# WestlyPark/StyleRenderer

Measured on AMD Instinct MI355X. Metric: generator fwd+bwd images/sec at 256^2, higher is better.
Workload: dtype f32

## Files before the change

### stylerenderer_amd/csrc/fused_elem.hip

```cpp
#include "common.h"

namespace {

constexpr int EB = 256;
constexpr int ECHUNK = EB * 16;

__device__ __forceinline__ void block_sum2(float& a, float& b, float* lds8) {
    a = sr_wave_sum(a);
    b = sr_wave_sum(b);
    const int lane = threadIdx.x & 63, wave = threadIdx.x >> 6;
    if (lane == 0) { lds8[wave] = a; lds8[4 + wave] = b; }
    __syncthreads();
    if (threadIdx.x == 0) {
        a = (lds8[0] + lds8[1]) + (lds8[2] + lds8[3]);
        b = (lds8[4] + lds8[5]) + (lds8[6] + lds8[7]);
    }
}

template <bool REF>
__global__ __launch_bounds__(EB) void k_nba_fwd(float* __restrict__ y, const float* __restrict__ x,
                                                const float* __restrict__ noise,
                                                const float* __restrict__ noise_w,
                                                const float* __restrict__ bias,
                                                const float* __restrict__ ref, float alpha, float scale,
// ... 114 lines not shown
}

template <bool SCALE_OUT, bool VEC>
__global__ __launch_bounds__(EB) void k_rowdot(float* __restrict__ partial, float* __restrict__ out,
                                               const float* __restrict__ a, const float* __restrict__ b,
                                               const float* __restrict__ s, int64_t inner, int chunks,
                                               const float* __restrict__ rdiv) {
    __shared__ float lds8[8];
    const int64_t row = blockIdx.y;
    const int64_t off = (int64_t)blockIdx.x * ECHUNK;
    const int64_t remain = inner - off;
    const int n = (int)(remain < ECHUNK ? remain : ECHUNK);
    const float sc = SCALE_OUT ? s[row] : 1.0f;
    float acc = 0.0f, dummy = 0.0f;
    if (VEC) {
        const float4* as = reinterpret_cast<const float4*>(a + row * inner + off);
        const float4* bs = reinterpret_cast<const float4*>(b + row * inner + off);
        float4* os = SCALE_OUT ? reinterpret_cast<float4*>(out + row * inner + off) : nullptr;
        for (int i = threadIdx.x; i < n / 4; i += EB) {
            const float4 x = as[i], y = bs[i];
            acc += (x.x * y.x + x.y * y.y) + (x.z * y.z + x.w * y.w);
            if (SCALE_OUT) os[i] = make_float4(y.x * sc, y.y * sc, y.z * sc, y.w * sc);
        }
    } else {
        const float* as = a + row * inner + off;
        const float* bs = b + row * inner + off;
        float* os = SCALE_OUT ? out + row * inner + off : nullptr;
#pragma unroll 4
        for (int i = threadIdx.x; i < n; i += EB) {
            const float x = as[i], y = bs[i];
            acc += x * y;
            if (SCALE_OUT) os[i] = y * sc;
        }
    }
    block_sum2(acc, dummy, lds8);
    if (threadIdx.x == 0) partial[row * chunks + blockIdx.x] = rdiv ? acc / rdiv[row] : acc;
}

__global__ __launch_bounds__(64) void k_rowdot_finish(float* __restrict__ dots,
                                                      const float* __restrict__ partial, int chunks,
                                                      const float* __restrict__ rdiv = nullptr) {
    const int64_t row = blockIdx.x;
    float acc = 0.0f;
    for (int i = threadIdx.x; i < chunks; i += 64) acc += partial[row * chunks + i];
    acc = sr_wave_sum(acc);
    if (threadIdx.x == 0) dots[row] = rdiv ? acc / rdiv[row] : acc;
}

inline bool vec_ok(int64_t inner, const void* p0, const void* p1, const void* p2, const void* p3) {
    const uintptr_t m = (uintptr_t)p0 | (uintptr_t)p1 | (uintptr_t)p2 | (uintptr_t)p3;
    return inner % 4 == 0 && (m & 15) == 0;
}

}

extern "C" int sr_noise_bias_act(float* y, const float* x, const float* noise, const float* noise_w,
                                 const float* bias, const float* ref, float alpha, float scale,
                                 int64_t n, int64_t c, int64_t inner, int64_t noise_bstride,
                                 sr_stream_t stream) {
    if (n < 0 || c < 0 || inner < 0) return SR_EINVAL;
    if (n * c * inner == 0) return SR_OK;
    if (!y || !x || (noise && !noise_w) || n * c > 65535) return SR_EINVAL;
    if (!vec_ok(inner, y, x, noise, ref) || (noise && noise_bstride % 4 != 0)) return SR_EINVAL;
    const int chunks = (int)sr_ceil_div(inner, ECHUNK);
    const dim3 grid(chunks, (unsigned)(n * c));
    hipStream_t st = sr_stream(stream);
    if (ref)
        hipLaunchKernelGGL(k_nba_fwd<true>, grid, dim3(EB), 0, st, y, x, noise, noise_w, bias, ref, alpha,
                           scale, (int)c, inner, noise_bstride);
    else
        hipLaunchKernelGGL(k_nba_fwd<false>, grid, dim3(EB), 0, st, y, x, noise, noise_w, bias, ref, alpha,
                           scale, (int)c, inner, noise_bstride);
    return sr_launch_status();
}

extern "C" int64_t sr_noise_bias_act_bwd_scratch_floats(int64_t n, int64_t c, int64_t inner) {
    if (n <= 0 || c <= 0 || inner <= 0) return 2;
    return 2 * n * c * sr_ceil_div(inner, ECHUNK) + c + 2;
}

extern "C" int sr_noise_bias_act_bwd(float* gx, float* gbias, float* gnoise_w, const float* gy,
                                     const float* out, const float* noise, float alpha, float scale,
                                     int64_t n, int64_t c, int64_t inner, int64_t noise_bstride,
                                     float* scratch, sr_stream_t stream) {
    if (n < 0 || c < 0 || inner < 0) return SR_EINVAL;
    if (n * c * inner == 0) return SR_OK;
    if (!gx || !gy || !out || !scratch || n * c > 65535) return SR_EINVAL;
    if (!vec_ok(inner, gx, gy, out, noise) || (noise && noise_bstride % 4 != 0)) return SR_EINVAL;
    const int chunks = (int)sr_ceil_div(inner, ECHUNK);
    hipStream_t st = sr_stream(stream);
    hipLaunchKernelGGL(k_nba_bwd<false>, dim3(chunks, (unsigned)(n * c)), dim3(EB), 0, st, gx, scratch, gy, out,
                       noise, alpha, scale, (int)c, inner, noise_bstride, chunks, (const float*)nullptr,
                       (const float*)nullptr, 0.0f, 0.0f, (float*)nullptr);
    float* chan_nw = scratch + 2 * n * c * (int64_t)chunks;
    if (gbias) {
        hipLaunchKernelGGL(k_nba_finish, dim3((unsigned)c), dim3(64), 0, st, gbias, chan_nw, scratch, n, (int)c,
                           chunks);
        if (noise && gnoise_w)
            hipLaunchKernelGGL(k_nba_finish2, dim3(1), dim3(64), 0, st, gnoise_w, chan_nw, (int)c);
    }
    return sr_launch_status();
}

int sr_nba_finish_launch(float* gbias, float* gnoise_w, float* rowdot, const float* partial, const float* dot_partial,
                         float* chan_nw, int64_t n, int64_t c, int chunks, bool has_noise, hipStream_t st) {
    if (gbias) {
        hipLaunchKernelGGL(k_nba_finish, dim3((unsigned)c), dim3(64), 0, st, gbias, chan_nw, partial, n, (int)c, chunks);
        if (has_noise && gnoise_w)
            hipLaunchKernelGGL(k_nba_finish2, dim3(1), dim3(64), 0, st, gnoise_w, chan_nw, (int)c);
    }
    if (rowdot) hipLaunchKernelGGL(k_rowdot_finish, dim3((unsigned)(n * c)), dim3(64), 0, st, rowdot, dot_partial, chunks);
    return sr_launch_status();
}

extern "C" int64_t sr_noise_bias_act_bwd_dot_scratch_floats(int64_t n, int64_t c, int64_t inner) {
    if (n <= 0 || c <= 0 || inner <= 0) return 3;
    return 3 * n * c * sr_ceil_div(inner, ECHUNK) + c + 2;
}

extern "C" int sr_noise_bias_act_bwd_dot(float* gx, float* gbias, float* gnoise_w, float* rowdot, const float* gy,
                                         const float* out, const float* noise, const float* noise_w,
                                         const float* bias, float alpha, float scale, int64_t n, int64_t c,
                                         int64_t inner, int64_t noise_bstride, float* scratch,
                                         sr_stream_t stream) {
    if (n < 0 || c < 0 || inner < 0) return SR_EINVAL;
    if (n * c * inner == 0) return SR_OK;
    if (!gx || !gy || !out || !scratch || !rowdot || n * c > 65535 || (noise && !noise_w) || scale == 0.0f ||
        alpha == 0.0f)
        return SR_EINVAL;
    if (!vec_ok(inner, gx, gy, out, noise) || (noise && noise_bstride % 4 != 0)) return SR_EINVAL;
    const int chunks = (int)sr_ceil_div(inner, ECHUNK);
    hipStream_t st = sr_stream(stream);
    float* dot_scratch = scratch + 2 * n * c * (int64_t)chunks;
    float* chan_nw = dot_scratch + n * c * (int64_t)chunks;
    float* dot_partial = chunks == 1 ? rowdot : dot_scratch;
    hipLaunchKernelGGL(k_nba_bwd<true>, dim3(chunks, (unsigned)(n * c)), dim3(EB), 0, st, gx, scratch, gy, out, noise,
                       alpha, scale, (int)c, inner, noise_bstride, chunks, noise_w, bias, 1.0f / scale,
                       1.0f / (alpha * scale), dot_partial);
    if (gbias) {
        hipLaunchKernelGGL(k_nba_finish, dim3((unsigned)c), dim3(64), 0, st, gbias, chan_nw, scratch, n, (int)c, chunks);
        if (noise && gnoise_w)
            hipLaunchKernelGGL(k_nba_finish2, dim3(1), dim3(64), 0, st, gnoise_w, chan_nw, (int)c);
    }
    if (chunks > 1)
        hipLaunchKernelGGL(k_rowdot_finish, dim3((unsigned)(n * c)), dim3(64), 0, st, rowdot, dot_partial, chunks);
    return sr_launch_status();
}

namespace {

constexpr int APIX = EB * 4;

__global__ __launch_bounds__(EB) void k_nba_aff_fwd(float* __restrict__ y, const float* __restrict__ x,
                                                    const float* __restrict__ amap, const float* __restrict__ smap,
                                                    int64_t map_bstride, const float* __restrict__ noise,
                                                    const float* __restrict__ noise_w,
                                                    const float* __restrict__ bias, float alpha, float scale, int c,
                                                    int64_t inner, int64_t noise_bstride, int cgroup) {
    const int64_t b = blockIdx.y;
    const int64_t p = (int64_t)blockIdx.x * APIX + threadIdx.x * 4;
    if (p >= inner) return;
    const int c0 = blockIdx.z * cgroup, c1 = (c0 + cgroup < c) ? c0 + cgroup : c;
    const float4 a = *reinterpret_cast<const float4*>(amap + b * map_bstride + p);
    const float4 sft = *reinterpret_cast<const float4*>(smap + b * map_bstride + p);
    const float nw = noise ? noise_w[0] : 0.0f;
    float4 nz = make_float4(0.f, 0.f, 0.f, 0.f);
    if (noise) nz = *reinterpret_cast<const float4*>(noise + b * noise_bstride + p);
    nz.x *= nw; nz.y *= nw; nz.z *= nw; nz.w *= nw;
    for (int ch = c0; ch < c1; ++ch) {
        const int64_t o = (b * c + ch) * inner + p;
        float4 v = *reinterpret_cast<const float4*>(x + o);
        const float bb = bias ? bias[ch] : 0.0f;
        v.x = v.x * a.x + sft.x; v.y = v.y * a.y + sft.y; v.z = v.z * a.z + sft.z; v.w = v.w * a.w + sft.w;
        if (noise) { v.x += nz.x; v.y += nz.y; v.z += nz.z; v.w += nz.w; }
        v.x += bb; v.y += bb; v.z += bb; v.w += bb;
        float4 r;
        r.x = ((v.x > 0.0f) ? v.x : v.x * alpha) * scale;
        r.y = ((v.y > 0.0f) ? v.y : v.y * alpha) * scale;
        r.z = ((v.z > 0.0f) ? v.z : v.z * alpha) * scale;
        r.w = ((v.w > 0.0f) ? v.w : v.w * alpha) * scale;
        *reinterpret_cast<float4*>(y + o) = r;
    }
}

__global__ __launch_bounds__(EB) void k_nba_aff_bwd(float* __restrict__ gx, float* __restrict__ gamap,
                                                    float* __restrict__ gsmap, float* __restrict__ partial,
                                                    const float* __restrict__ gy, const float* __restrict__ out,
                                                    const float* __restrict__ x, const float* __restrict__ amap,
                                                    int64_t map_bstride, const float* __restrict__ noise,
                                                    float alpha, float scale, int c, int64_t inner,
                                                    int64_t noise_bstride, int chunks, int cgroup,
                                                    int64_t plane) {
    const int64_t b = blockIdx.y;
    const int64_t p = (int64_t)blockIdx.x * APIX + threadIdx.x * 4;
    const bool live = p < inner;
    const int c0 = blockIdx.z * cgroup, c1 = (c0 + cgroup < c) ? c0 + cgroup : c;
    gamap += (int64_t)blockIdx.z * plane;
    gsmap += (int64_t)blockIdx.z * plane;
    const int lane = threadIdx.x & 63, wave = threadIdx.x >> 6;
// ... 506 lines not shown
    }
    const int lane = threadIdx.x & 63, wave = threadIdx.x >> 6;
#pragma unroll
    for (int k = 0; k < CH; ++k)
#pragma unroll
        for (int j = 0; j < N; ++j) {
            const float r = sr_wave_sum(acc[k][j]);
            if (lane == 0) lds[k][j * 4 + wave] = r;
        }
    if (sum_g) {
#pragma unroll
        for (int j = 0; j < N; ++j) {
            const float r = sr_wave_sum(ag[j]);
            if (lane == 0) lds_g[j * 4 + wave] = r;
        }
    }
    __syncthreads();
    if (sum_g && threadIdx.x >= 64 && threadIdx.x < 64 + N) {
        const int j = threadIdx.x - 64;
        gsum[(b * chunks + blockIdx.x) * N + j] = (lds_g[j * 4] + lds_g[j * 4 + 1]) + (lds_g[j * 4 + 2] + lds_g[j * 4 + 3]);
    }
    if (threadIdx.x < CH * N) {
        const int k = threadIdx.x / N, j = threadIdx.x % N;
        const float r = (lds[k][j * 4] + lds[k][j * 4 + 1]) + (lds[k][j * 4 + 2] + lds[k][j * 4 + 3]);
        if (dws) dws[(b * N + j) * C + (row0 + k - b * C)] = r;
        else partial[((row0 + k) * chunks + blockIdx.x) * N + j] = r;
    }
}

__global__ __launch_bounds__(64) void k_smallconv_dw_finish(float* __restrict__ dws,
                                                            const float* __restrict__ partial, int C, int N,
                                                            int chunks, int64_t rows) {
    const int64_t row = blockIdx.x;
    if (row >= rows) return;
    const int64_t b = row / C, c = row % C;
    for (int j = 0; j < N; ++j) {
        float acc = 0.0f;
        for (int i = threadIdx.x; i < chunks; i += 64) acc += partial[(row * chunks + i) * N + j];
        acc = sr_wave_sum(acc);
        if (threadIdx.x == 0) dws[(b * N + j) * C + c] = acc;
    }
}

__global__ __launch_bounds__(64) void k_smallconv_gb_finish(float* __restrict__ gb, const float* __restrict__ gsum, int N,
                                                            int entries) {
    for (int j = 0; j < N; ++j) {
        float acc = 0.0f;
        for (int i = threadIdx.x; i < entries; i += 64) acc += gsum[(int64_t)i * N + j];
        acc = sr_wave_sum(acc);
        if (threadIdx.x == 0) gb[j] = acc;
    }
}

inline bool smallconv_ok(int64_t B, int64_t C, int64_t N, int64_t hw, const void* a, const void* b2) {
    return B > 0 && B <= 65535 && C > 0 && C <= 4096 && N >= 1 && N <= SC_MAXN && hw % 4 == 0 &&
           (((uintptr_t)a | (uintptr_t)b2) & 15) == 0;
}

}

#define SR_SMALLCONV_DISPATCH(KERNEL, ...)                                   \
    switch (N) {                                                             \
        case 1: hipLaunchKernelGGL(KERNEL<1>, __VA_ARGS__); break;           \
        case 2: hipLaunchKernelGGL(KERNEL<2>, __VA_ARGS__); break;           \
        case 3: hipLaunchKernelGGL(KERNEL<3>, __VA_ARGS__); break;           \
        default: hipLaunchKernelGGL(KERNEL<4>, __VA_ARGS__); break;          \
    }

extern "C" int sr_smallconv_fwd(float* out, const float* x, const float* ws, const float* bias, int64_t B,
                                int64_t C, int64_t N, int64_t hw, sr_stream_t stream) {
    if (!out || !x || !ws || !smallconv_ok(B, C, N, hw, out, x)) return SR_EINVAL;
    const int64_t hw4 = hw / 4;
    const dim3 grid((unsigned)sr_ceil_div(hw4, 64), (unsigned)B);
    hipStream_t st = sr_stream(stream);
    const bool wide = sr_ceil_div(hw4, 64) * B < 1024 && C >= 64;
#define SR_SMALLCONV_FWD(NN)                                                                                          \
    if (wide) hipLaunchKernelGGL((k_smallconv_fwd<NN, 16>), grid, dim3(1024), 0, st, out, x, ws, bias, (int)C, hw4);  \
    else hipLaunchKernelGGL((k_smallconv_fwd<NN, 4>), grid, dim3(256), 0, st, out, x, ws, bias, (int)C, hw4);
    switch (N) {
        case 1: SR_SMALLCONV_FWD(1) break;
        case 2: SR_SMALLCONV_FWD(2) break;
        case 3: SR_SMALLCONV_FWD(3) break;
        default: SR_SMALLCONV_FWD(4) break;
    }
#undef SR_SMALLCONV_FWD
    return sr_launch_status();
}

extern "C" int sr_smallconv_dx_add(float* dx, const float* g, const float* ws, const float* addend, int64_t B, int64_t C,
                                   int64_t N, int64_t hw, sr_stream_t stream);

extern "C" int sr_smallconv_dx(float* dx, const float* g, const float* ws, int64_t B, int64_t C, int64_t N,
                               int64_t hw, sr_stream_t stream) {
    return sr_smallconv_dx_add(dx, g, ws, nullptr, B, C, N, hw, stream);
}

extern "C" int sr_smallconv_dx_add(float* dx, const float* g, const float* ws, const float* addend, int64_t B, int64_t C,
                                   int64_t N, int64_t hw, sr_stream_t stream) {
    if (!dx || !g || !ws || !smallconv_ok(B, C, N, hw, dx, g) || ((uintptr_t)addend & 15)) return SR_EINVAL;
    const int64_t hw4 = hw / 4;
    const int64_t wgs = sr_ceil_div(hw4, 256) * B;
    int64_t groups = sr_ceil_div(2048, wgs);
    if (groups > sr_ceil_div(C, 8)) groups = sr_ceil_div(C, 8);
    if (groups < 1) groups = 1;
    const int cgroup = (int)(sr_ceil_div(sr_ceil_div(C, groups), 8) * 8);
    const dim3 grid((unsigned)sr_ceil_div(hw4, 256), (unsigned)B, (unsigned)sr_ceil_div(C, cgroup));
    const size_t lds = (size_t)N * C * sizeof(float);
    hipStream_t st = sr_stream(stream);
    SR_SMALLCONV_DISPATCH(k_smallconv_dx, grid, dim3(256), lds, st, dx, g, ws, (int)C, hw4, addend, cgroup);
    return sr_launch_status();
}

extern "C" int64_t sr_smallconv_dw_scratch_floats(int64_t B, int64_t C, int64_t N, int64_t hw) {
    if (B <= 0 || C <= 0 || N <= 0 || hw <= 0) return 1;
    return B * C * sr_ceil_div(hw, ECHUNK) * N + B * sr_ceil_div(hw, ECHUNK) * N + 1;
}

extern "C" int sr_smallconv_dw_bias(float* dws, float* gb, const float* g, const float* x, int64_t B, int64_t C, int64_t N,
                                    int64_t hw, float* scratch, sr_stream_t stream) {
    if (!dws || !g || !x || !scratch || !smallconv_ok(B, C, N, hw, g, x) || B * C > 65535) return SR_EINVAL;
    const int chunks = (int)sr_ceil_div(hw, ECHUNK);
    hipStream_t st = sr_stream(stream);
    float* direct = chunks == 1 ? dws : nullptr;
    float* gsum = gb ? scratch + B * C * chunks * N : nullptr;
    if (C % 4 == 0) {
        const dim3 grid((unsigned)chunks, (unsigned)(B * C / 4));
        switch (N) {
            case 1: hipLaunchKernelGGL((k_smallconv_dw<1, 4>), grid, dim3(256), 0, st, scratch, g, x, (int)C, hw, chunks, direct, gsum); break;
            case 2: hipLaunchKernelGGL((k_smallconv_dw<2, 4>), grid, dim3(256), 0, st, scratch, g, x, (int)C, hw, chunks, direct, gsum); break;
            case 3: hipLaunchKernelGGL((k_smallconv_dw<3, 4>), grid, dim3(256), 0, st, scratch, g, x, (int)C, hw, chunks, direct, gsum); break;
            default: hipLaunchKernelGGL((k_smallconv_dw<4, 4>), grid, dim3(256), 0, st, scratch, g, x, (int)C, hw, chunks, direct, gsum); break;
        }
    } else {
        const dim3 grid((unsigned)chunks, (unsigned)(B * C));
        switch (N) {
            case 1: hipLaunchKernelGGL((k_smallconv_dw<1, 1>), grid, dim3(256), 0, st, scratch, g, x, (int)C, hw, chunks, direct, gsum); break;
            case 2: hipLaunchKernelGGL((k_smallconv_dw<2, 1>), grid, dim3(256), 0, st, scratch, g, x, (int)C, hw, chunks, direct, gsum); break;
            case 3: hipLaunchKernelGGL((k_smallconv_dw<3, 1>), grid, dim3(256), 0, st, scratch, g, x, (int)C, hw, chunks, direct, gsum); break;
            default: hipLaunchKernelGGL((k_smallconv_dw<4, 1>), grid, dim3(256), 0, st, scratch, g, x, (int)C, hw, chunks, direct, gsum); break;
        }
    }
    if (chunks > 1)
        hipLaunchKernelGGL(k_smallconv_dw_finish, dim3((unsigned)(B * C)), dim3(64), 0, st, dws, scratch, (int)C,
                           (int)N, chunks, B * C);
    if (gb)
        hipLaunchKernelGGL(k_smallconv_gb_finish, dim3(1), dim3(64), 0, st, gb, gsum, (int)N, (int)(B * chunks));
    return sr_launch_status();
}

extern "C" int sr_smallconv_dw(float* dws, const float* g, const float* x, int64_t B, int64_t C, int64_t N,
                               int64_t hw, float* scratch, sr_stream_t stream) {
    return sr_smallconv_dw_bias(dws, nullptr, g, x, B, C, N, hw, scratch, stream);
}

namespace {

template <int N, int CH>
__global__ __launch_bounds__(EB) void k_fork_nba_bwd(float* __restrict__ gpre, float* __restrict__ partial,
                                                     float* __restrict__ dot_partial, float* __restrict__ dw_partial,
                                                     float* __restrict__ dws, float* __restrict__ gsum,
                                                     const float* __restrict__ addend, const float* __restrict__ y,
                                                     const float* __restrict__ g, const float* __restrict__ ws,
                                                     const float* __restrict__ noise, const float* __restrict__ noise_w,
                                                     const float* __restrict__ bias, float alpha, float scale,
                                                     float inv_pos, float inv_neg, int C, int64_t hw,
                                                     int64_t noise_bstride, int chunks) {
    __shared__ float lds_nba[CH][2][8];
    __shared__ float lds[CH][4 * SC_MAXN];
    __shared__ float lds_g[4 * SC_MAXN];
    const int64_t row0 = (int64_t)blockIdx.y * CH;
    const int64_t b = row0 / C;
    const int c0 = (int)(row0 - b * C);
    const int64_t off = (int64_t)blockIdx.x * ECHUNK;
    const int64_t remain = hw - off;
    const int n4 = (int)((remain < ECHUNK ? remain : ECHUNK) / 4);
    const float4* ns = noise ? reinterpret_cast<const float4*>(noise + b * noise_bstride + off) : nullptr;
    const float nw = noise ? noise_w[0] : 0.0f;
    float w[CH][N], bb[CH];
#pragma unroll
    for (int k = 0; k < CH; ++k) {
        bb[k] = bias ? bias[c0 + k] : 0.0f;
#pragma unroll
        for (int j = 0; j < N; ++j) w[k][j] = ws[(b * N + j) * C + c0 + k];
    }
    float acc[CH][N], sb[CH], sn[CH], sd[CH], ag[N];
#pragma unroll
    for (int k = 0; k < CH; ++k) {
        sb[k] = sn[k] = sd[k] = 0.0f;
#pragma unroll
        for (int j = 0; j < N; ++j) acc[k][j] = 0.0f;
    }
#pragma unroll
    for (int j = 0; j < N; ++j) ag[j] = 0.0f;
    const bool sum_g = gsum != nullptr && c0 == 0;
    for (int i = threadIdx.x; i < n4; i += EB) {
        float4 gg[N], a[CH], o[CH];
#pragma unroll
        for (int j = 0; j < N; ++j) gg[j] = reinterpret_cast<const float4*>(g + (b * N + j) * hw + off)[i];
#pragma unroll
        for (int k = 0; k < CH; ++k) {
// ... 70 lines not shown
    if (threadIdx.x < CH * N) {
        const int k = threadIdx.x / N, j = threadIdx.x % N;
        const float r = (lds[k][j * 4] + lds[k][j * 4 + 1]) + (lds[k][j * 4 + 2] + lds[k][j * 4 + 3]);
        if (dws) dws[(b * N + j) * C + (c0 + k)] = r;
        else dw_partial[((row0 + k) * chunks + blockIdx.x) * N + j] = r;
    }
}

constexpr int FORK_CH = 4;

inline int64_t fork_nba_floats(int64_t B, int64_t C, int64_t hw) {
    const int64_t n = 3 * B * C * sr_ceil_div(hw, ECHUNK) + C + 2;
    return n + (n & 1);
}

}

extern "C" int64_t sr_fork_nba_bwd_scratch_floats(int64_t B, int64_t C, int64_t N, int64_t hw) {
    if (B <= 0 || C <= 0 || N <= 0 || hw <= 0) return 4;
    return fork_nba_floats(B, C, hw) + B * C * sr_ceil_div(hw, ECHUNK) * N + B * sr_ceil_div(hw, ECHUNK) * N + 1;
}

extern "C" int sr_fork_nba_bwd(float* gpre, float* gbias, float* gnoise_w, float* rowdot, float* dws, float* gb_rgb,
                               const float* g_above, const float* y, const float* g_rgb, const float* ws,
                               const float* noise, const float* noise_w, const float* bias, float alpha, float scale,
                               int64_t B, int64_t C, int64_t N, int64_t hw, int64_t noise_bstride, float* scratch,
                               sr_stream_t stream) {
    if (!gpre || !rowdot || !dws || !y || !g_rgb || !ws || !scratch || (noise && !noise_w) || scale == 0.0f ||
        alpha == 0.0f)
        return SR_EINVAL;
    if (!smallconv_ok(B, C, N, hw, g_rgb, y) || hw <= 0 || C % FORK_CH != 0 || B * C > 65535) return SR_EINVAL;
    if (!vec_ok(hw, gpre, g_above, y, noise) || (noise && noise_bstride % 4 != 0) || gpre == g_above) return SR_EINVAL;
    const int chunks = (int)sr_ceil_div(hw, ECHUNK);
    hipStream_t st = sr_stream(stream);
    const int64_t rows = B * C;
    float* dot_scratch = scratch + 2 * rows * chunks;
    float* chan_nw = dot_scratch + rows * chunks;
    float* dw_scratch = scratch + fork_nba_floats(B, C, hw);
    float* dot_partial = chunks == 1 ? rowdot : dot_scratch;
    float* direct = chunks == 1 ? dws : nullptr;
    float* gsum = gb_rgb ? dw_scratch + rows * chunks * N : nullptr;
    const dim3 grid((unsigned)chunks, (unsigned)(rows / FORK_CH));
#define SR_FORK_NBA(NN)                                                                                                    \
    hipLaunchKernelGGL((k_fork_nba_bwd<NN, FORK_CH>), grid, dim3(EB), 0, st, gpre, scratch, dot_partial, dw_scratch, direct,  \
                       gsum, g_above, y, g_rgb, ws, noise, noise_w, bias, alpha, scale, 1.0f / scale,                       \
                       1.0f / (alpha * scale), (int)C, hw, noise_bstride, chunks)
    switch (N) {
        case 1: SR_FORK_NBA(1); break;
        case 2: SR_FORK_NBA(2); break;
        case 3: SR_FORK_NBA(3); break;
        default: SR_FORK_NBA(4); break;
    }
#undef SR_FORK_NBA
    if (gbias) {
        hipLaunchKernelGGL(k_nba_finish, dim3((unsigned)C), dim3(64), 0, st, gbias, chan_nw, scratch, B, (int)C, chunks);
        if (noise && gnoise_w)
            hipLaunchKernelGGL(k_nba_finish2, dim3(1), dim3(64), 0, st, gnoise_w, chan_nw, (int)C);
    }
    if (chunks > 1) {
        hipLaunchKernelGGL(k_rowdot_finish, dim3((unsigned)rows), dim3(64), 0, st, rowdot, dot_partial, chunks);
        hipLaunchKernelGGL(k_smallconv_dw_finish, dim3((unsigned)rows), dim3(64), 0, st, dws, dw_scratch, (int)C, (int)N,
                           chunks, rows);
    }
    if (gb_rgb)
        hipLaunchKernelGGL(k_smallconv_gb_finish, dim3(1), dim3(64), 0, st, gb_rgb, gsum, (int)N, (int)(B * chunks));
    return sr_launch_status();
}

namespace {

__global__ __launch_bounds__(256) void k_modrows_fwd(float* __restrict__ ws, const float* __restrict__ w,
                                                     const float* __restrict__ s, float scale, int B, int N, int C) {
    const int64_t i = (int64_t)blockIdx.x * 256 + threadIdx.x;
    if (i >= (int64_t)B * N * C) return;
    const int c = (int)(i % C);
    const int j = (int)((i / C) % N);
    const int b = (int)(i / ((int64_t)C * N));
    ws[i] = (w[(int64_t)j * C + c] * scale) * s[(int64_t)b * C + c];
}

__global__ __launch_bounds__(256) void k_modrows_bwd(float* __restrict__ gs, float* __restrict__ gw,
                                                     const float* __restrict__ dws, const float* __restrict__ w,
                                                     const float* __restrict__ s, float scale, int B, int N, int C) {
    const int c = blockIdx.x * 256 + threadIdx.x;
    if (c >= C) return;
    const int r = blockIdx.y;
    if (r < B) {
        if (!gs) return;
        float acc = 0.0f;
        for (int j = 0; j < N; ++j) acc += dws[((int64_t)r * N + j) * C + c] * (w[(int64_t)j * C + c] * scale);
        gs[(int64_t)r * C + c] = acc;
    } else {
        if (!gw) return;
        const int j = r - B;
        float acc = 0.0f;
#pragma unroll 4
        for (int b = 0; b < B; ++b) acc += dws[((int64_t)b * N + j) * C + c] * s[(int64_t)b * C + c];
        gw[(int64_t)j * C + c] = acc * scale;
    }
}

}

extern "C" int sr_modrows_fwd(float* ws, const float* w, const float* s, float scale, int64_t B, int64_t N, int64_t C,
                              sr_stream_t stream) {
    if (B == 0 || N == 0 || C == 0) return SR_OK;
    if (!ws || !w || !s || B < 0 || N < 0 || C < 0) return SR_EINVAL;
    if (B > 65535 || N > 65535 || C > (1 << 20)) return SR_ERANGE;
    const int64_t total = B * N * C;
    hipLaunchKernelGGL(k_modrows_fwd, dim3((unsigned)sr_ceil_div(total, 256)), dim3(256), 0, sr_stream(stream), ws, w, s,
                       scale, (int)B, (int)N, (int)C);
    return sr_launch_status();
}

extern "C" int sr_modrows_bwd(float* gs, float* gw, const float* dws, const float* w, const float* s, float scale,
                              int64_t B, int64_t N, int64_t C, sr_stream_t stream) {
    if (N == 0 || C == 0 || (!gs && !gw)) return SR_OK;
    if (!dws || !w || !s || B < 0 || N < 0 || C < 0) return SR_EINVAL;
    if (B > 65535 || N > 65535 || B + N > 65535 || C > (1 << 20)) return SR_ERANGE;
// ... 96 lines not shown
```

### stylerenderer_amd/csrc/weight_prep.hip

```cpp
#include "common.h"

namespace {

template <int KK>
__global__ __launch_bounds__(256) void k_wprep(float* __restrict__ wt, float* __restrict__ wsq,
                                               const float* __restrict__ w, float scale, int Co, int Ci,
                                               int ld) {
    const int co = blockIdx.x * 64 + (threadIdx.x & 63);
    const int ci = blockIdx.y * 4 + (threadIdx.x >> 6);
    if (ci >= Ci || co >= ld) return;
    float v[KK];
    float sq = 0.0f;
    if (co < Co) {
        const float* src = w + ((int64_t)co * Ci + ci) * KK;
#pragma unroll
        for (int t = 0; t < KK; ++t) {
            v[t] = src[t] * scale;
            sq += v[t] * v[t];
        }
    } else {
#pragma unroll
        for (int t = 0; t < KK; ++t) v[t] = 0.0f;
    }
#pragma unroll
    for (int t = 0; t < KK; ++t) wt[((int64_t)t * Ci + ci) * ld + co] = v[t];
    if (wsq && co < Co) wsq[(int64_t)ci * Co + co] = sq;
}

template <int KK>
__global__ __launch_bounds__(256) void k_wprep_bwd(float* __restrict__ gw, const float* __restrict__ gwt,
                                                   const float* __restrict__ gwsq,
                                                   const float* __restrict__ w, float scale, int Co,
                                                   int Ci, int ldg) {
    __shared__ float tile[16][16 * KK + 1];
    const int co0 = blockIdx.x * 16, ci0 = blockIdx.y * 16;
    const int row_floats = 16 * KK;
    if (gwsq) {
        for (int e = threadIdx.x; e < 16 * row_floats; e += 256) {
            const int r = e / row_floats, q = e % row_floats;
            const int co = co0 + r, ci = ci0 + q / KK;
            tile[r][q] = (co < Co && ci < Ci) ? w[((int64_t)co * Ci + ci0) * KK + q] : 0.0f;
        }
        __syncthreads();
    }
    const int lco = threadIdx.x & 15, lci = threadIdx.x >> 4;
    const int co = co0 + lco, ci = ci0 + lci;
    const bool ok = co < Co && ci < Ci;
    const float q2 = (gwsq && ok) ? 2.0f * scale * scale * gwsq[(int64_t)ci * Co + co] : 0.0f;
#pragma unroll
    for (int t = 0; t < KK; ++t) {
        float g = (gwt && ok) ? scale * gwt[((int64_t)t * Ci + ci) * ldg + co] : 0.0f;
        if (gwsq) g += q2 * tile[lco][lci * KK + t];
        tile[lco][lci * KK + t] = g;
    }
    __syncthreads();
    for (int e = threadIdx.x; e < 16 * row_floats; e += 256) {
        const int r = e / row_floats, q = e % row_floats;
        const int oco = co0 + r, oci = ci0 + q / KK;
        if (oco < Co && oci < Ci) gw[((int64_t)oco * Ci + ci0) * KK + q] = tile[r][q];
    }
}

__global__ __launch_bounds__(256) void k_wadjoint(float* __restrict__ out, const float* __restrict__ in,
                                                  int C, int N, int ldn, int ldc, int KK, int flip) {
    __shared__ float tile[32][33];
    const int t = blockIdx.z;
    const int tA = flip ? KK - 1 - t : t;
    const int c0 = blockIdx.x * 32, n0 = blockIdx.y * 32;
    const int tx = threadIdx.x & 31, ty = threadIdx.x >> 5;
#pragma unroll
    for (int r = ty; r < 32; r += 8) {
        const int c = c0 + r, n = n0 + tx;
        tile[r][tx] = (c < C && n < N) ? in[((int64_t)t * C + c) * ldn + n] : 0.0f;
    }
    __syncthreads();
#pragma unroll
    for (int r = ty; r < 32; r += 8) {
        const int n = n0 + r, c = c0 + tx;
        if (n < N && c < ldc) out[((int64_t)tA * N + n) * ldc + c] = tile[tx][r];
    }
}


constexpr int SR_WB_MAX = 48;

struct WPrepBatch {
    float* wt[SR_WB_MAX];
    float* wsq[SR_WB_MAX];
    const float* w[SR_WB_MAX];
    float scale[SR_WB_MAX];
    int co[SR_WB_MAX], ci[SR_WB_MAX], ld[SR_WB_MAX], kk[SR_WB_MAX];
    int first[SR_WB_MAX + 1];
    int n;
};

__device__ __forceinline__ int wb_item(const int* first, int n, int bid) {
    int it = 0;
    while (it + 1 < n && bid >= first[it + 1]) ++it;
    return it;
}

template <int KK>
__device__ __forceinline__ void wprep_tile(float* __restrict__ wt, float* __restrict__ wsq, const float* __restrict__ w,
                                           float scale, int Co, int Ci, int ld, int bx, int by) {
    const int co = bx * 64 + (threadIdx.x & 63);
    const int ci = by * 4 + (threadIdx.x >> 6);
    if (ci >= Ci || co >= ld) return;
    float v[KK];
    float sq = 0.0f;
    if (co < Co) {
        const float* src = w + ((int64_t)co * Ci + ci) * KK;
#pragma unroll
        for (int t = 0; t < KK; ++t) {
// ... 26 lines not shown
};

__global__ __launch_bounds__(256) void k_wadjoint_batch(const WAdjBatch b) {
    __shared__ float tile[32][33];
    const int it = wb_item(b.first, b.n, blockIdx.x);
    int local = blockIdx.x - b.first[it];
    const int C = b.C[it], N = b.N[it], ldn = b.ldn[it], ldc = b.ldc[it], KK = b.KK[it];
    const int gx = (ldc + 31) / 32, gy = (N + 31) / 32;
    const int bx = local % gx;
    local /= gx;
    const int by = local % gy, t = local / gy;
    const int tA = b.flip[it] ? KK - 1 - t : t;
    const float* __restrict__ in = b.in[it];
    float* __restrict__ out = b.out[it];
    const int c0 = bx * 32, n0 = by * 32;
    const int tx = threadIdx.x & 31, ty = threadIdx.x >> 5;
#pragma unroll
    for (int r = ty; r < 32; r += 8) {
        const int c = c0 + r, n = n0 + tx;
        tile[r][tx] = (c < C && n < N) ? in[((int64_t)t * C + c) * ldn + n] : 0.0f;
    }
    __syncthreads();
#pragma unroll
    for (int r = ty; r < 32; r += 8) {
        const int n = n0 + r, c = c0 + tx;
        if (n < N && c < ldc) out[((int64_t)tA * N + n) * ldc + c] = tile[tx][r];
    }
}

}

extern "C" int sr_weight_prep(float* wt, float* wsq, const float* w, float scale, int64_t Co, int64_t Ci,
                              int ksize, int64_t ld, sr_stream_t stream) {
    if (Co <= 0 || Ci <= 0 || !wt || !w || ld < Co || (ld & 3)) return SR_EINVAL;
    if (Co > (1 << 20) || Ci > (1 << 20)) return SR_ERANGE;
    const dim3 grid((unsigned)sr_ceil_div(ld, 64), (unsigned)sr_ceil_div(Ci, 4));
    hipStream_t st = sr_stream(stream);
    if (ksize == 3)
        hipLaunchKernelGGL(k_wprep<9>, grid, dim3(256), 0, st, wt, wsq, w, scale, (int)Co, (int)Ci, (int)ld);
    else if (ksize == 1)
        hipLaunchKernelGGL(k_wprep<1>, grid, dim3(256), 0, st, wt, wsq, w, scale, (int)Co, (int)Ci, (int)ld);
    else
        return SR_EINVAL;
    return sr_launch_status();
}

extern "C" int sr_weight_prep_bwd(float* gw, const float* gwt, const float* gwsq, const float* w,
                                  float scale, int64_t Co, int64_t Ci, int ksize, int64_t ldg,
                                  sr_stream_t stream) {
    if (Co <= 0 || Ci <= 0 || !gw || (!gwt && !gwsq) || (gwsq && !w) || (gwt && ldg < Co)) return SR_EINVAL;
    if (Co > (1 << 20) || Ci > (1 << 20)) return SR_ERANGE;
    const dim3 grid((unsigned)sr_ceil_div(Co, 16), (unsigned)sr_ceil_div(Ci, 16));
    hipStream_t st = sr_stream(stream);
    if (ksize == 3)
        hipLaunchKernelGGL(k_wprep_bwd<9>, grid, dim3(256), 0, st, gw, gwt, gwsq, w, scale, (int)Co, (int)Ci,
                           (int)ldg);
    else if (ksize == 1)
        hipLaunchKernelGGL(k_wprep_bwd<1>, grid, dim3(256), 0, st, gw, gwt, gwsq, w, scale, (int)Co, (int)Ci,
                           (int)ldg);
    else
        return SR_EINVAL;
    return sr_launch_status();
}

extern "C" int sr_weight_adjoint(float* out, const float* in, int64_t taps, int64_t C, int64_t N, int64_t ldn,
                                 int64_t ldc, int flip, sr_stream_t stream) {
    if (taps <= 0 || C <= 0 || N <= 0 || !out || !in || ldn < N || ldc < C) return SR_EINVAL;
    if (taps > 65535 || sr_ceil_div(N, 32) > 65535) return SR_ERANGE;
    const dim3 grid((unsigned)sr_ceil_div(ldc, 32), (unsigned)sr_ceil_div(N, 32), (unsigned)taps);
    hipLaunchKernelGGL(k_wadjoint, grid, dim3(256), 0, sr_stream(stream), out, in, (int)C, (int)N, (int)ldn,
                       (int)ldc, (int)taps, flip);
    return sr_launch_status();
}

extern "C" int sr_weight_prep_batch(int n, float* const* wt, float* const* wsq, const float* const* w,
                                    const float* scale, const int64_t* Co, const int64_t* Ci, const int* ksize,
                                    const int64_t* ld, sr_stream_t stream) {
    if (n < 0 || (n > 0 && (!wt || !wsq || !w || !scale || !Co || !Ci || !ksize || !ld))) return SR_EINVAL;
    hipStream_t st = sr_stream(stream);
    for (int base = 0; base < n; base += SR_WB_MAX) {
        WPrepBatch b;
        b.n = n - base < SR_WB_MAX ? n - base : SR_WB_MAX;
        int64_t total = 0;
        for (int i = 0; i < b.n; ++i) {
            const int g = base + i;
            if (Co[g] <= 0 || Ci[g] <= 0 || !wt[g] || !w[g] || ld[g] < Co[g] || (ld[g] & 3) || (ksize[g] != 1 && ksize[g] != 3))
                return SR_EINVAL;
            if (Co[g] > (1 << 20) || Ci[g] > (1 << 20)) return SR_ERANGE;
            b.wt[i] = wt[g]; b.wsq[i] = wsq[g]; b.w[i] = w[g]; b.scale[i] = scale[g];
            b.co[i] = (int)Co[g]; b.ci[i] = (int)Ci[g]; b.ld[i] = (int)ld[g]; b.kk[i] = ksize[g] * ksize[g];
            b.first[i] = (int)total;
            total += sr_ceil_div(ld[g], 64) * sr_ceil_div(Ci[g], 4);
            if (total > 0x7FFFFFFFLL) return SR_ERANGE;
        }
        b.first[b.n] = (int)total;
        if (total > 0) hipLaunchKernelGGL(k_wprep_batch, dim3((unsigned)total), dim3(256), 0, st, b);
    }
    return sr_launch_status();
}

extern "C" int sr_weight_adjoint_batch(int n, float* const* out, const float* const* in, const int64_t* taps,
                                       const int64_t* C, const int64_t* N, const int64_t* ldn, const int64_t* ldc,
                                       const int* flip, sr_stream_t stream) {
    if (n < 0 || (n > 0 && (!out || !in || !taps || !C || !N || !ldn || !ldc || !flip))) return SR_EINVAL;
    hipStream_t st = sr_stream(stream);
    for (int base = 0; base < n; base += SR_WB_MAX) {
// ... 20 lines not shown
```

Measured before the change: 634.1.

## Fuse backward tail reductions into one kernel and widen weight-prep backward tiles

Replaces the separate small finish kernels (bias sums, noise-weight sum, row dot finish, smallconv dw and rgb-bias finish) with a single multi-role kernel whose workgroup ranges are dispatched by block index. This cuts per-layer launch count in the backward pass. It also adds a wider weight-prep backward kernel (64 Co by 4 Ci tiles) that loads and stores the weight gradient with float4 accesses to improve coalescing. Both paths are on by default and can be disabled through environment variables, and the fused kernel reorders float reductions.

```diff
diff --git a/stylerenderer_amd/csrc/fused_elem.hip b/stylerenderer_amd/csrc/fused_elem.hip
--- a/stylerenderer_amd/csrc/fused_elem.hip
+++ b/stylerenderer_amd/csrc/fused_elem.hip
@@ -190,6 +190,15 @@
     return inner % 4 == 0 && (m & 15) == 0;
 }
 
+enum TailEntry { TAIL_NBA, TAIL_BLUR, TAIL_SMALLCONV };
+struct TailSums {
+    float* gbias; float* gnoise_w; bool has_noise; const float* partial; float* chan_nw; int64_t n; int64_t c;
+    float* rowdot; const float* dot_partial;
+    float* dws; const float* dw_partial; int N; float* gb_rgb; const float* gsum;
+    int chunks;
+};
+int tail_sums_launch(TailEntry entry, const TailSums& s, hipStream_t st);
+
 }
 
 extern "C" int sr_noise_bias_act(float* y, const float* x, const float* noise, const float* noise_w,
@@ -231,24 +240,16 @@
                        noise, alpha, scale, (int)c, inner, noise_bstride, chunks, (const float*)nullptr,
                        (const float*)nullptr, 0.0f, 0.0f, (float*)nullptr);
     float* chan_nw = scratch + 2 * n * c * (int64_t)chunks;
-    if (gbias) {
-        hipLaunchKernelGGL(k_nba_finish, dim3((unsigned)c), dim3(64), 0, st, gbias, chan_nw, scratch, n, (int)c,
-                           chunks);
-        if (noise && gnoise_w)
-            hipLaunchKernelGGL(k_nba_finish2, dim3(1), dim3(64), 0, st, gnoise_w, chan_nw, (int)c);
-    }
-    return sr_launch_status();
+    const TailSums sums{gbias, gnoise_w, noise != nullptr, scratch, chan_nw, n, c, nullptr, nullptr,
+                        nullptr, nullptr, 0, nullptr, nullptr, chunks};
+    return tail_sums_launch(TAIL_NBA, sums, st);
 }
 
 int sr_nba_finish_launch(float* gbias, float* gnoise_w, float* rowdot, const float* partial, const float* dot_partial,
                          float* chan_nw, int64_t n, int64_t c, int chunks, bool has_noise, hipStream_t st) {
-    if (gbias) {
-        hipLaunchKernelGGL(k_nba_finish, dim3((unsigned)c), dim3(64), 0, st, gbias, chan_nw, partial, n, (int)c, chunks);
-        if (has_noise && gnoise_w)
-            hipLaunchKernelGGL(k_nba_finish2, dim3(1), dim3(64), 0, st, gnoise_w, chan_nw, (int)c);
-    }
-    if (rowdot) hipLaunchKernelGGL(k_rowdot_finish, dim3((unsigned)(n * c)), dim3(64), 0, st, rowdot, dot_partial, chunks);
-    return sr_launch_status();
+    const TailSums sums{gbias, gnoise_w, has_noise, partial, chan_nw, n, c, rowdot, dot_partial,
+                        nullptr, nullptr, 0, nullptr, nullptr, chunks};
+    return tail_sums_launch(TAIL_BLUR, sums, st);
 }
 
 extern "C" int64_t sr_noise_bias_act_bwd_dot_scratch_floats(int64_t n, int64_t c, int64_t inner) {
@@ -275,14 +276,9 @@
     hipLaunchKernelGGL(k_nba_bwd<true>, dim3(chunks, (unsigned)(n * c)), dim3(EB), 0, st, gx, scratch, gy, out, noise,
                        alpha, scale, (int)c, inner, noise_bstride, chunks, noise_w, bias, 1.0f / scale,
                        1.0f / (alpha * scale), dot_partial);
-    if (gbias) {
-        hipLaunchKernelGGL(k_nba_finish, dim3((unsigned)c), dim3(64), 0, st, gbias, chan_nw, scratch, n, (int)c, chunks);
-        if (noise && gnoise_w)
-            hipLaunchKernelGGL(k_nba_finish2, dim3(1), dim3(64), 0, st, gnoise_w, chan_nw, (int)c);
-    }
-    if (chunks > 1)
-        hipLaunchKernelGGL(k_rowdot_finish, dim3((unsigned)(n * c)), dim3(64), 0, st, rowdot, dot_partial, chunks);
-    return sr_launch_status();
+    const TailSums sums{gbias, gnoise_w, noise != nullptr, scratch, chan_nw, n, c, chunks > 1 ? rowdot : nullptr,
+                        dot_partial, nullptr, nullptr, 0, nullptr, nullptr, chunks};
+    return tail_sums_launch(TAIL_NBA, sums, st);
 }
 
 namespace {
@@ -895,6 +891,149 @@
     }
 }
 
+constexpr int TF_WAVES = 16;
+constexpr int TF_MAXC = 4096;
+constexpr int TF_NW_UNROLL = 8;
+
+struct TailFinish {
+    int wg_bias, wg_nw, wg_dot, wg_dw, wg_gb;
+    float* gb; float* gnw; const float* partial;
+    int64_t n, rows;
+    int c, chunks;
+    float* dots; const float* dot_partial;
+    float* dws; const float* dw_partial;
+    float* gb_rgb; const float* gsum;
+    int N, entries;
+};
+
+__global__ __launch_bounds__(TF_WAVES * 64) void k_tail_finish(const TailFinish p) {
+    __shared__ float shares[TF_MAXC];
+    const int lane = threadIdx.x & 63, wave = threadIdx.x >> 6;
+    int bid = blockIdx.x;
+    if (bid < p.wg_bias) {
+        const int ch = bid * TF_WAVES + wave;
+        if (ch >= p.c) return;
+        float acc = 0.0f;
+        const int64_t total = p.n * p.chunks;
+        for (int64_t i = lane; i < total; i += 64) {
+            const int64_t s = i / p.chunks, k = i % p.chunks;
+            acc += p.partial[((s * p.c + ch) * p.chunks + k) * 2];
+        }
+        acc = sr_wave_sum(acc);
+        if (lane == 0) p.gb[ch] = acc;
+        return;
+    }
+    bid -= p.wg_bias;
+    if (bid < p.wg_nw) {
+        const int64_t total = p.n * p.chunks;
+        for (int ch0 = wave; ch0 < p.c; ch0 += TF_WAVES * TF_NW_UNROLL) {
+            float acc[TF_NW_UNROLL];
+#pragma unroll
+            for (int u = 0; u < TF_NW_UNROLL; ++u) acc[u] = 0.0f;
+            for (int64_t i = lane; i < total; i += 64) {
+                const int64_t s = i / p.chunks, k = i % p.chunks;
+#pragma unroll
+                for (int u = 0; u < TF_NW_UNROLL; ++u) {
+                    const int ch = ch0 + u * TF_WAVES;
+                    if (ch < p.c) acc[u] += p.partial[((s * p.c + ch) * p.chunks + k) * 2 + 1];
+                }
+            }
+#pragma unroll
+            for (int u = 0; u < TF_NW_UNROLL; ++u) {
+                const int ch = ch0 + u * TF_WAVES;
+                const float r = sr_wave_sum(acc[u]);
+                if (lane == 0 && ch < p.c) shares[ch] = r;
+            }
+        }
+        __syncthreads();
+        if (wave == 0) {
+            float acc = 0.0f;
+            for (int i = lane; i < p.c; i += 64) acc += shares[i];
+            acc = sr_wave_sum(acc);
+            if (lane == 0) p.gnw[0] = acc;
+        }
+        return;
+    }
+    bid -= p.wg_nw;
+    if (bid < p.wg_dot) {
+        const int64_t row = (int64_t)bid * TF_WAVES + wave;
+        if (row >= p.rows) return;
+        float acc = 0.0f;
+        for (int i = lane; i < p.chunks; i += 64) acc += p.dot_partial[row * p.chunks + i];
+        acc = sr_wave_sum(acc);
+        if (lane == 0) p.dots[row] = acc;
+        return;
+    }
+    bid -= p.wg_dot;
+    if (bid < p.wg_dw) {
+        const int64_t row = (int64_t)bid * TF_WAVES + wave;
+        if (row >= p.rows) return;
+        const int64_t b = row / p.c, c = row % p.c;
+        for (int j = 0; j < p.N; ++j) {
+            float acc = 0.0f;
+            for (int i = lane; i < p.chunks; i += 64) acc += p.dw_partial[(row * p.chunks + i) * p.N + j];
+            acc = sr_wave_sum(acc);
+            if (lane == 0) p.dws[(b * p.N + j) * p.c + c] = acc;
+        }
+        return;
+    }
+    if (wave < p.N) {
+        const int j = wave;
+        float acc = 0.0f;
+        for (int i = lane; i < p.entries; i += 64) acc += p.gsum[(int64_t)i * p.N + j];
+        acc = sr_wave_sum(acc);
+        if (lane == 0) p.gb_rgb[j] = acc;
+    }
+}
+
+inline int tail_finish_mode() {
+    static const int mode = [] {
+        const char* e = std::getenv("SR_TAIL_FINISH");
+        if (!e) return 1;
+        return e[0] == '0' ? 0 : (e[0] == 'a' ? 2 : 1);
+    }();
+    return mode;
+}
+
+int tail_sums_launch(TailEntry entry, const TailSums& s, hipStream_t st) {
+    const int mode = s.c <= TF_MAXC && s.N <= TF_WAVES ? tail_finish_mode() : 0;
+    const bool fused = mode == 2 || (mode == 1 && entry != TAIL_SMALLCONV);
+    const bool fuse_dot = mode == 2 || entry == TAIL_NBA;
+    const int64_t rows = s.n * s.c;
+    const bool want_nw = s.gbias && s.has_noise && s.gnoise_w;
+    if (fused) {
+        TailFinish p{};
+        p.n = s.n; p.rows = rows; p.c = (int)s.c; p.chunks = s.chunks; p.N = s.N;
+        p.gb = s.gbias; p.gnw = s.gnoise_w; p.partial = s.partial;
+        p.dots = s.rowdot; p.dot_partial = s.dot_partial;
+        p.dws = s.dws; p.dw_partial = s.dw_partial;
+        p.gb_rgb = s.gb_rgb; p.gsum = s.gsum; p.entries = (int)(s.n * s.chunks);
+        p.wg_bias = s.gbias ? (int)sr_ceil_div(s.c, TF_WAVES) : 0;
+        p.wg_nw = want_nw ? 1 : 0;
+        p.wg_dot = s.rowdot && fuse_dot ? (int)sr_ceil_div(rows, TF_WAVES) : 0;
+        p.wg_dw = s.dws ? (int)sr_ceil_div(rows, TF_WAVES) : 0;
+        p.wg_gb = s.gb_rgb ? 1 : 0;
+        const int wgs = p.wg_bias + p.wg_nw + p.wg_dot + p.wg_dw + p.wg_gb;
+        if (wgs > 0) hipLaunchKernelGGL(k_tail_finish, dim3((unsigned)wgs), dim3(TF_WAVES * 64), 0, st, p);
+        if (s.rowdot && !fuse_dot)
+            hipLaunchKernelGGL(k_rowdot_finish, dim3((unsigned)rows), dim3(64), 0, st, s.rowdot, s.dot_partial, s.chunks);
+        return sr_launch_status();
+    }
+    if (s.gbias) {
+        hipLaunchKernelGGL(k_nba_finish, dim3((unsigned)s.c), dim3(64), 0, st, s.gbias, s.chan_nw, s.partial, s.n, (int)s.c,
+                           s.chunks);
+        if (want_nw) hipLaunchKernelGGL(k_nba_finish2, dim3(1), dim3(64), 0, st, s.gnoise_w, s.chan_nw, (int)s.c);
+    }
+    if (s.rowdot)
+        hipLaunchKernelGGL(k_rowdot_finish, dim3((unsigned)rows), dim3(64), 0, st, s.rowdot, s.dot_partial, s.chunks);
+    if (s.dws)
+        hipLaunchKernelGGL(k_smallconv_dw_finish, dim3((unsigned)rows), dim3(64), 0, st, s.dws, s.dw_partial, (int)s.c,
+                           s.N, s.chunks, rows);
+    if (s.gb_rgb)
+        hipLaunchKernelGGL(k_smallconv_gb_finish, dim3(1), dim3(64), 0, st, s.gb_rgb, s.gsum, s.N, (int)(s.n * s.chunks));
+    return sr_launch_status();
+}
+
 inline bool smallconv_ok(int64_t B, int64_t C, int64_t N, int64_t hw, const void* a, const void* b2) {
     return B > 0 && B <= 65535 && C > 0 && C <= 4096 && N >= 1 && N <= SC_MAXN && hw % 4 == 0 &&
            (((uintptr_t)a | (uintptr_t)b2) & 15) == 0;
@@ -983,12 +1122,9 @@
             default: hipLaunchKernelGGL((k_smallconv_dw<4, 1>), grid, dim3(256), 0, st, scratch, g, x, (int)C, hw, chunks, direct, gsum); break;
         }
     }
-    if (chunks > 1)
-        hipLaunchKernelGGL(k_smallconv_dw_finish, dim3((unsigned)(B * C)), dim3(64), 0, st, dws, scratch, (int)C,
-                           (int)N, chunks, B * C);
-    if (gb)
-        hipLaunchKernelGGL(k_smallconv_gb_finish, dim3(1), dim3(64), 0, st, gb, gsum, (int)N, (int)(B * chunks));
-    return sr_launch_status();
+    const TailSums sums{nullptr, nullptr, false, nullptr, nullptr, B, C, nullptr, nullptr,
+                        chunks > 1 ? dws : nullptr, scratch, (int)N, gb, gsum, chunks};
+    return tail_sums_launch(TAIL_SMALLCONV, sums, st);
 }
 
 extern "C" int sr_smallconv_dw(float* dws, const float* g, const float* x, int64_t B, int64_t C, int64_t N,
@@ -1165,19 +1301,9 @@
         default: SR_FORK_NBA(4); break;
     }
 #undef SR_FORK_NBA
-    if (gbias) {
-        hipLaunchKernelGGL(k_nba_finish, dim3((unsigned)C), dim3(64), 0, st, gbias, chan_nw, scratch, B, (int)C, chunks);
-        if (noise && gnoise_w)
-            hipLaunchKernelGGL(k_nba_finish2, dim3(1), dim3(64), 0, st, gnoise_w, chan_nw, (int)C);
-    }
-    if (chunks > 1) {
-        hipLaunchKernelGGL(k_rowdot_finish, dim3((unsigned)rows), dim3(64), 0, st, rowdot, dot_partial, chunks);
-        hipLaunchKernelGGL(k_smallconv_dw_finish, dim3((unsigned)rows), dim3(64), 0, st, dws, dw_scratch, (int)C, (int)N,
-                           chunks, rows);
-    }
-    if (gb_rgb)
-        hipLaunchKernelGGL(k_smallconv_gb_finish, dim3(1), dim3(64), 0, st, gb_rgb, gsum, (int)N, (int)(B * chunks));
-    return sr_launch_status();
+    const TailSums sums{gbias, gnoise_w, noise != nullptr, scratch, chan_nw, B, C, chunks > 1 ? rowdot : nullptr,
+                        dot_partial, chunks > 1 ? dws : nullptr, dw_scratch, (int)N, gb_rgb, gsum, chunks};
+    return tail_sums_launch(TAIL_NBA, sums, st);
 }
 
 namespace {
diff --git a/stylerenderer_amd/csrc/weight_prep.hip b/stylerenderer_amd/csrc/weight_prep.hip
--- a/stylerenderer_amd/csrc/weight_prep.hip
+++ b/stylerenderer_amd/csrc/weight_prep.hip
@@ -59,6 +59,53 @@
         const int oco = co0 + r, oci = ci0 + q / KK;
         if (oco < Co && oci < Ci) gw[((int64_t)oco * Ci + ci0) * KK + q] = tile[r][q];
     }
+}
+
+constexpr int WW_CO = 64, WW_CI = 4;
+
+template <int KK>
+__global__ __launch_bounds__(256) void k_wprep_bwd_wide(float* __restrict__ gw, const float* __restrict__ gwt,
+                                                        const float* __restrict__ gwsq, const float* __restrict__ w,
+                                                        float scale, int Co, int Ci, int ldg) {
+    constexpr int ROW = WW_CI * KK, ROW4 = ROW / 4;
+    __shared__ float tile[WW_CO][ROW + 1];
+    const int co0 = blockIdx.x * WW_CO, ci0 = blockIdx.y * WW_CI;
+    const int lco = threadIdx.x & 63, lci = threadIdx.x >> 6;
+    const int co = co0 + lco, ci = ci0 + lci;
+    const bool ok = co < Co;
+    float g[KK];
+#pragma unroll
+    for (int t = 0; t < KK; ++t) g[t] = (gwt && ok) ? gwt[((int64_t)t * Ci + ci) * ldg + co] : 0.0f;
+    const float sq = (gwsq && ok) ? gwsq[(int64_t)ci * Co + co] : 0.0f;
+    if (gwsq) {
+        for (int e = threadIdx.x; e < WW_CO * ROW4; e += 256) {
+            const int r = e / ROW4, q = e % ROW4;
+            float4 v = make_float4(0.0f, 0.0f, 0.0f, 0.0f);
+            if (co0 + r < Co) v = *reinterpret_cast<const float4*>(w + ((int64_t)(co0 + r) * Ci + ci0) * KK + 4 * q);
+            tile[r][q] = v.x; tile[r][ROW4 + q] = v.y; tile[r][2 * ROW4 + q] = v.z; tile[r][3 * ROW4 + q] = v.w;
+        }
+        __syncthreads();
+    }
+    const float q2 = (gwsq && ok) ? 2.0f * scale * scale * sq : 0.0f;
+#pragma unroll
+    for (int t = 0; t < KK; ++t) {
+        const int x = lci * KK + t, idx = (x & 3) * ROW4 + (x >> 2);
+        float v = (gwt && ok) ? scale * g[t] : 0.0f;
+        if (gwsq) v += q2 * tile[lco][idx];
+        tile[lco][idx] = v;
+    }
+    __syncthreads();
+    for (int e = threadIdx.x; e < WW_CO * ROW4; e += 256) {
+        const int r = e / ROW4, q = e % ROW4;
+        if (co0 + r < Co)
+            *reinterpret_cast<float4*>(gw + ((int64_t)(co0 + r) * Ci + ci0) * KK + 4 * q) =
+                make_float4(tile[r][q], tile[r][ROW4 + q], tile[r][2 * ROW4 + q], tile[r][3 * ROW4 + q]);
+    }
+}
+
+inline bool wprep_bwd_wide_enabled() {
+    static const bool enabled = !sr_env_off("SR_WPREP_BWD_WIDE");
+    return enabled;
 }
 
 __global__ __launch_bounds__(256) void k_wadjoint(float* __restrict__ out, const float* __restrict__ in,
@@ -191,6 +238,17 @@
     if (Co > (1 << 20) || Ci > (1 << 20)) return SR_ERANGE;
     const dim3 grid((unsigned)sr_ceil_div(Co, 16), (unsigned)sr_ceil_div(Ci, 16));
     hipStream_t st = sr_stream(stream);
+    if ((ksize == 3 || ksize == 1) && wprep_bwd_wide_enabled() && Ci % WW_CI == 0 && Ci / WW_CI <= 65535 &&
+        sr_aligned16(gw) && (!gwsq || sr_aligned16(w))) {
+        const dim3 wgrid((unsigned)sr_ceil_div(Co, WW_CO), (unsigned)(Ci / WW_CI));
+        if (ksize == 3)
+            hipLaunchKernelGGL(k_wprep_bwd_wide<9>, wgrid, dim3(256), 0, st, gw, gwt, gwsq, w, scale, (int)Co, (int)Ci,
+                               (int)ldg);
+        else
+            hipLaunchKernelGGL(k_wprep_bwd_wide<1>, wgrid, dim3(256), 0, st, gw, gwt, gwsq, w, scale, (int)Co, (int)Ci,
+                               (int)ldg);
+        return sr_launch_status();
+    }
     if (ksize == 3)
         hipLaunchKernelGGL(k_wprep_bwd<9>, grid, dim3(256), 0, st, gw, gwt, gwsq, w, scale, (int)Co, (int)Ci,
                            (int)ldg);
```

Measured after the change: 634.3, median of 2. About the same (+0.0%).
